# AkshayJha22/Cross-Sectional-Momentum-Strategy-Replication-Backtesting-Framework

Measured on AMD Instinct MI355X. Metric: asset-periods backtested/sec (1/2/4/8 GPU) + % HBM peak BW; decile match %, higher is better.
Workload: dtype f64

## Files before the change

cross-sectional-momentum-strategy-replication-backtesting-framework_amd/csrc/signal.hip:

```cpp
#include "csm_common.h"
#include "scan.h"
#include "shard.h"


#define PROBE_M 8
#define PROBE_DEN 8
__device__ __forceinline__ bool tail_probe(const double* __restrict__ P,
                                           const int64_t* __restrict__ month_start, int T_m,
                                           int64_t N, int64_t T_d) {
  static_assert(PROBE_M == 8, "the month spacing is a shift");
  const int lane = threadIdx.x & 63;
  const int64_t cs = N / 128;
  double x[PROBE_M][2];
  bool in[PROBE_M];
#pragma unroll
  for (int i = 0; i < PROBE_M; ++i) {
    const int m = (int)(((int64_t)(2 * i + 1) * T_m) >> 4);
    const int64_t d0 = month_start[m] < 0 ? 0 : month_start[m];
    const int64_t d1 = month_start[m + 1] < T_d ? month_start[m + 1] : T_d;
    in[i] = d1 > d0;
#pragma unroll
    for (int j = 0; j < 2; ++j)
      x[i][j] = in[i] ? P[(d1 - 1) * N + (2 * lane + j) * cs] : 0.0;
  }
  int gaps = 0, tot = 0;
#pragma unroll
  for (int i = 0; i < PROBE_M; ++i)
#pragma unroll
    for (int j = 0; j < 2; ++j) {
      gaps += __popcll(__ballot(in[i] && !(x[i][j] == x[i][j])));
      tot += in[i] ? 64 : 0;
    }
  return gaps * PROBE_DEN <= tot;
}

struct HaloArgs {
  int H, F, before, after;
  uint8_t* flags;
};
#define HALO_BATCH 8
template <int MAXD, int VEC, int NBUF, int BW, bool SH, bool BL, int JC = 0, bool HALO = false>
__global__ __launch_bounds__(64 * BW) void k_signal(
    const double* __restrict__ P, const int64_t* __restrict__ month_start, int T_m, int64_t N,
    int J, int skip, double* __restrict__ PMo, double* __restrict__ R, double* __restrict__ M,
    double* __restrict__ NR, const double* __restrict__ carry, const double* __restrict__ next_pm,
    double* __restrict__ carry_out, int64_t T_d, uint16_t* __restrict__ IDS, HaloArgs ha,
    int probe) {
  static_assert(!HALO || (SH && VEC == 2), "the halo prologue: shard passes, paired lanes");
  if (probe && tail_probe(P, month_start, T_m, N, T_d)) return;
  typedef typename RowT<VEC>::T VT;
  extern __shared__ __attribute__((aligned(16))) double ring_lds[];
  const int W = J + skip;
  const int tid = threadIdx.x;
  const int64_t a0 = ((int64_t)blockIdx.x * 64 * BW + tid) * VEC;
  const bool live = a0 < N;
  const int RS = 64 * VEC * BW;
  ScanLane sl[VEC];
  int* shc = reinterpret_cast<int*>(ring_lds + W * RS);
#pragma unroll
  for (int k = 0; k < VEC; ++k) {
    scan_init(sl[k], ring_lds + VEC * tid + k, RS, W, HALO ? nullptr : carry, N, a0 + k, live);
    if (SH) {
      shc[VEC * tid + k] = 0;
      shc[RS + VEC * tid + k] = -1;
      shc[2 * RS + VEC * tid + k] = -1;
    }
  }
  double npmh[VEC];
  if constexpr (HALO) {
    constexpr int HU = HALO_BATCH;
    const int64_t* ms = month_start;
    const int H = ha.H, F = ha.F, HF = H + F;
    const int64_t as = live ? a0 : 0;
    const int lane = tid & 63, wv = tid >> 6;
    const int64_t aw = a0 - 2 * lane;
    double* hpw = ring_lds + (size_t)W * RS + (size_t)(3 * RS) / 2;
    uint16_t* wl = reinterpret_cast<uint16_t*>(hpw + HU * RS) + wv * (HU * 128);
    int nh[VEC], fv[VEC], lv[VEC];
#pragma unroll
    for (int c = 0; c < VEC; ++c) { nh[c] = 0; fv[c] = -1; lv[c] = -1; npmh[c] = absent_val(); }
    for (int j0 = 0; j0 < HF; j0 += HU) {
      double2 xl[HU];
#pragma unroll
// ... 162 lines not shown
      }
    }
  };
  static_assert(NBUF == 2 || NBUF == 4, "two or four month buffers");
  VT A[MAXD], B[MAXD];
  if (NBUF == 2) {
    load_month(A, 0);
    for (int m = 0; m < T_m; m += 2) {
      load_month(B, m + 1);
      process(A, m);
      load_month(A, m + 2);
      if (m + 1 < T_m) process(B, m + 1);
    }
  } else {
    VT C[MAXD], D[MAXD];
    load_month(A, 0);
    load_month(B, 1);
    load_month(C, 2);
    for (int m = 0; m < T_m; m += 4) {
      load_month(D, m + 3);
      process(A, m);
      load_month(A, m + 4);
      if (m + 1 < T_m) process(B, m + 1);
      load_month(B, m + 5);
      if (m + 2 < T_m) process(C, m + 2);
      load_month(C, m + 6);
      if (m + 3 < T_m) process(D, m + 3);
    }
  }
  if (live) {
#pragma unroll
    for (int k = 0; k < VEC; ++k) {
      if constexpr (HALO) {
        if (sl[k].prev >= 0)
          NR[(int64_t)sl[k].prev * N + a0 + k] = pending_finish(npmh[k], sl[k].psff);
      } else {
        scan_finish(sl[k], ring_lds + VEC * tid + k, RS, W, N, a0 + k, NR, next_pm,
                    SH ? nullptr : carry_out);
      }
      if (SH) {
        const int* q = shc + VEC * tid + k;
        carry_out[a0 + k] = (double)q[0];
        carry_out[N + a0 + k] = (double)sl[k].prev;
        carry_out[2 * N + a0 + k] = sl[k].psff;
        carry_out[3 * N + a0 + k] = (double)q[RS];
        carry_out[4 * N + a0 + k] = (double)q[2 * RS];
      }
    }
  }
}

#define TAIL_U 8
#define TAIL_BACK 3

template <int MAXD, int BW, int JC>
__global__ __launch_bounds__(64 * BW) void k_signal_tail(
    const double* __restrict__ P, const int64_t* __restrict__ month_start, int T_m, int64_t N,
    int J, int skip, double* __restrict__ PMo, double* __restrict__ R, double* __restrict__ M,
    double* __restrict__ NR, const double* __restrict__ carry, const double* __restrict__ next_pm,
    double* __restrict__ carry_out, int64_t T_d, uint16_t* __restrict__ IDS,
    int probe) {
  if (probe && !tail_probe(P, month_start, T_m, N, T_d)) return;
  extern __shared__ __attribute__((aligned(16))) double ring_lds[];
  constexpr int U = TAIL_U, RS = 64 * BW, WA = 64;
  const int W = J + skip;
  const int tid = threadIdx.x, lane = tid & 63, wv = tid >> 6;
  const int64_t a0 = (int64_t)blockIdx.x * RS + tid;
  const bool live = a0 < N;
  const int64_t as = live ? a0 : 0;
  const int64_t aw = a0 - lane;
  const int64_t* ms = month_start;
  double* hp = ring_lds + (size_t)W * RS;
  double* hpw = hp + WA * wv;
  uint16_t* wl = reinterpret_cast<uint16_t*>(hp + U * RS) + wv * (2 * U * WA);
  uint16_t* wl2 = wl + U * WA;
  ScanLane sl;
  scan_init(sl, ring_lds + tid, RS, W, carry, N, a0, live);
  if (aw >= N) return;

  auto month_rows = [&](int m, int64_t& d0, int64_t& d1) {
    d0 = ms[m];
    d1 = ms[m + 1];
    d0 = d0 < 0 ? 0 : d0;
    d1 = d1 < T_d ? d1 : T_d;
  };
  auto load_last = [&](double (&xl)[U], int m0) {
#pragma unroll
    for (int u = 0; u < U; ++u) {
      xl[u] = absent_val();
      if (m0 + u < T_m) {
        int64_t d0, d1;
        month_rows(m0 + u, d0, d1);
        if (d1 > d0) xl[u] = P[(d1 - 1) * N + as];
      }
    }
  };
  auto fold = [&](double y, double& x, bool& got, bool& p) {
    if (!got && y == y) { x = y; got = true; }
    p |= !is_absent(y);
  };
  constexpr int K = MAXD - 1;
  struct Walk {
    int item, u, col;
    int64_t d0, d1;
    bool act;
  };
  auto issue = [&](auto& xs, Walk& w, const uint16_t* list, int it, int n, int m0) {
    constexpr int KK = sizeof(xs) / sizeof(double);
    w.act = it < n;
    w.item = w.act ? (int)list[it] : 0;
    w.u = w.item / WA;
    w.col = w.item % WA;
    month_rows(m0 + w.u, w.d0, w.d1);
    const int64_t a = aw + w.col;
#pragma unroll
    for (int k = 0; k < KK; ++k) {
      const int64_t d = w.d1 - 2 - k;
      xs[k] = (w.act && d >= w.d0) ? P[d * N + a] : absent_val();
    }
  };
  auto finish_back = [&](const double (&xs)[TAIL_BACK], const Walk& w, int& nb) {
    bool p = true, got = false;
    double x = 0.0;
#pragma unroll
    for (int k = 0; k < TAIL_BACK; ++k) fold(xs[k], x, got, p);
    const bool more = w.act && !got && w.d1 - 2 - TAIL_BACK >= w.d0;
    if (w.act && !more) hpw[w.u * RS + w.col] = got ? x : qnan();
    const uint64_t mk = __ballot(more);
    if (more) wl2[nb + lane_prefix(mk)] = (uint16_t)w.item;
    nb += __popcll(mk);
  };
  auto finish_month = [&](const double (&xs)[K], const Walk& w) {
    bool p = !is_absent(hpw[w.u * RS + w.col]), got = false;
    double x = 0.0;
#pragma unroll
    for (int k = 0; k < K; ++k) fold(xs[k], x, got, p);
    if (w.act) hpw[w.u * RS + w.col] = got ? x : (p ? qnan() : absent_val());
  };
  auto walk_months = [&](int i0, int n, int m0) {
    double XS[K], XT[K];
    Walk wb, wc;
    const bool two = i0 + 64 < n;
    issue(XS, wb, wl2, i0 + lane, n, m0);
    if (two) issue(XT, wc, wl2, i0 + 64 + lane, n, m0);
    finish_month(XS, wb);
    if (two) finish_month(XT, wc);
  };

  double xa[U], xb[U];
  load_last(xa, 0);
  for (int m0 = 0; m0 < T_m; m0 += U) {
    load_last(xb, m0 + U);
    int na = 0, nb = 0;
#pragma unroll
    for (int u = 0; u < U; ++u) {
      hp[u * RS + tid] = xa[u];
      bool in = false;
      if (m0 + u < T_m) {
        int64_t d0, d1;
        month_rows(m0 + u, d0, d1);
        in = d1 > d0;
      }
      const double x = xa[u];
      const bool need = live && in && !(x == x);
      const bool nb_ = need && is_absent(x), na_ = need && !nb_;
      const uint64_t mka = __ballot(na_), mkb = __ballot(nb_);
      const int item = u * WA + lane;
      if (na_) wl[na + lane_prefix(mka)] = (uint16_t)item;
      if (nb_) wl2[nb + lane_prefix(mkb)] = (uint16_t)item;
      na += __popcll(mka);
      nb += __popcll(mkb);
    }
    __builtin_amdgcn_wave_barrier();
    if (na + nb > 0) {
      double xs[TAIL_BACK];
      Walk wa;
      int db = nb < 128 ? nb : 128;
      issue(xs, wa, wl, lane, na, m0);
      walk_months(0, db, m0);
      finish_back(xs, wa, nb);
      for (int it0 = 64; it0 < na; it0 += 64) {
        issue(xs, wa, wl, it0 + lane, na, m0);
        finish_back(xs, wa, nb);
      }
      __builtin_amdgcn_wave_barrier();
      for (; db < nb; db += 128) walk_months(db, nb, m0);
    }
    __builtin_amdgcn_wave_barrier();
#pragma unroll 1
    for (int u = 0; u < U; ++u) {
      const int m = m0 + u;
      if (m >= T_m) break;
      if (!live) continue;
      const double pm = hp[u * RS + tid];
      if (PMo) PMo[(int64_t)m * N + a0] = pm;
      const double mom = scan_step<JC>(sl, pm, m, ring_lds + tid, RS, W, J, N, a0, R, M, NR);
      if (IDS) IDS[(int64_t)m * N + a0] = (uint16_t)csm_fid(mom);
    }
    __builtin_amdgcn_wave_barrier();
#pragma unroll
    for (int u = 0; u < U; ++u) xa[u] = xb[u];
  }
  if (live) scan_finish(sl, ring_lds + tid, RS, W, N, a0, NR, next_pm, carry_out);
}

static int g_tune_signal_vec = 2;
static int g_tune_signal_bwf = 0;
static int g_tune_signal_tail = 2;
static int g_tune_signal_j12 = 1;
#define SIGNAL_BWF_MIN_N (180 * 512)
static const TuneKnob g_knobs[] = {
    {"signal_vec", &g_tune_signal_vec, [](int v) { return v == 1 || v == 2; }},
    {"signal_bwf", &g_tune_signal_bwf, [](int v) { return v == 0 || v == 1 || v == 4; }},
    {"signal_j12", &g_tune_signal_j12, [](int v) { return v == 0 || v == 1; }},
    {"signal_tail", &g_tune_signal_tail, [](int v) { return v >= 0 && v <= 2; }},
};
int csm_tune_signal(const char* key, int value) { return tune_set(g_knobs, key, value); }

int signal_launch(csm_ctx* ctx, const char* who, const double* P, int64_t T_d, int64_t N,
                  const int64_t* month_start, int32_t T_m, int32_t max_month_days, int32_t J,
                  int32_t skip, double* PM, double* R, double* M, double* NR, const double* carry,
                  const double* next_pm, double* carry_out, bool sh, uint16_t* ids,
                  const HaloArgs* halo) {
  int r = prep(ctx);
  if (r) return r;
  if (sh && (!PM || !carry_out || T_m < 1))
    return set_err(ctx, CSM_E_INVAL, "%s: a shard pass needs PM and state, and at least one month",
                   who);
  if (!P || !month_start || !M || !NR || N <= 0 || T_d < 0 || T_m < 0 || J < 1 || skip < 0 ||
      J + skip > 256 || max_month_days < 1)
    return set_err(ctx, CSM_E_INVAL, "%s: bad arguments (N=%lld T_m=%d J=%d skip=%d)", who,
                   (long long)N, T_m, J, skip);
  if (max_month_days > 32)
    return set_err(ctx, CSM_E_INVAL, "%s: months longer than 32 days are not supported "
                   "(use csm_month_end + csm_momentum)", who);
  if (T_m == 0) return CSM_OK;
  if (T_d == 0)
    return set_err(ctx, CSM_E_INVAL, "%s: %d months and no day row", who, T_m);
  const int W = J + skip;
  const bool can2 = (N % 2 == 0) && aligned16(P) && (!PM || aligned16(PM)) && aligned16(M) &&
                    aligned16(NR) && (!R || aligned16(R));
  const int vec = (g_tune_signal_vec == 1 || !can2) ? 1 : 2;
  const size_t tlds = (size_t)(W + TAIL_U) * 128 * sizeof(double) + (size_t)2 * TAIL_U * 128 * sizeof(uint16_t);
  int tail = (!sh && !halo && can2 && tlds <= 160 * 1024) ? g_tune_signal_tail : 0;
  if (tail == 2 && N < (int64_t)SIGNAL_BWF_MIN_N) tail = 1;
  int probe_ = tail == 2;
  if (tail != 0) {
    const bool d23 = max_month_days <= 23, j12 = J == 12;
    const void* fn =
        d23 ? (j12 ? (const void*)k_signal_tail<23, 2, 12> : (const void*)k_signal_tail<23, 2, 0>)
            : (j12 ? (const void*)k_signal_tail<32, 2, 12> : (const void*)k_signal_tail<32, 2, 0>);
    if (tlds > 65536)
      HIP_CHECK(ctx, hipFuncSetAttribute(fn, hipFuncAttributeMaxDynamicSharedMemorySize, (int)tlds));
    const unsigned blocks = (unsigned)((N + 127) / 128);
    int T_m_ = T_m, J_ = J, skip_ = skip;
    int64_t N_ = N, T_d_ = T_d;
    void* args[] = {(void*)&P, (void*)&month_start, &T_m_, &N_, &J_, &skip_, (void*)&PM, (void*)&R,
                    (void*)&M, (void*)&NR, (void*)&carry, (void*)&next_pm, (void*)&carry_out, &T_d_,
                    (void*)&ids, &probe_};
    HIP_CHECK(ctx, hipLaunchKernel(fn, dim3(blocks), dim3(128), args, tlds, ctx->stream));
    LAUNCH_CHECK(ctx, who);
    if (tail == 1) return CSM_OK;
  }
  const bool fits4 = vec == 2 && max_month_days <= 23 && N * 8 * 32 < ((int64_t)1 << 31);
  const bool wide4 = fits4 && (g_tune_signal_bwf == 4 ||
                               (g_tune_signal_bwf == 0 && N >= (int64_t)SIGNAL_BWF_MIN_N));
  const int bw = wide4 ? 4 : 1;
  const size_t lds = (size_t)W * 64 * vec * bw * sizeof(double) +
                     (sh ? (size_t)3 * 64 * vec * bw * sizeof(int) : 0) +
                     (halo ? (size_t)HALO_BATCH * 64 * vec * bw * sizeof(double) +
                             (size_t)bw * HALO_BATCH * 128 * sizeof(uint16_t) : 0);
  const unsigned blocks = (unsigned)((N / vec + 64 * bw - 1) / (64 * bw));
  const void* fn = nullptr;
#define SIG1(V, SH_)                                                                            \
  (max_month_days <= 23 && V == 2 ? (const void*)k_signal<23, V, 4, 1, SH_, false>              \
   : max_month_days <= 24         ? (const void*)k_signal<24, V, 4, 1, SH_, false>              \
                                  : (const void*)k_signal<32, V, 4, 1, SH_, false>)
  const bool j12 = sh && J == 12 && g_tune_signal_j12;
  if (halo && !(sh && wide4))
    return set_err(ctx, CSM_E_INVAL, "%s: the fused halo prologue runs in the wide shard kernel "
                   "(even N >= %d, months of <= 23 days); use csm_shard_halo + "
                   "csm_signal_shard_halo", who, SIGNAL_BWF_MIN_N);
  if (halo)
    fn = j12 ? (const void*)k_signal<23, 2, 2, 4, true, true, 12, true>
             : (const void*)k_signal<23, 2, 2, 4, true, true, 0, true>;
  else if (wide4 && j12)
    fn = (const void*)k_signal<23, 2, 2, 4, true, true, 12>;
  else if (wide4)
    fn = sh ? (const void*)k_signal<23, 2, 2, 4, true, true> : (const void*)k_signal<23, 2, 2, 4, false, true>;
  else if (vec == 2)
    fn = sh ? SIG1(2, true) : SIG1(2, false);
  else
    fn = sh ? SIG1(1, true) : SIG1(1, false);
#undef SIG1
  if (lds > 65536)
    HIP_CHECK(ctx, hipFuncSetAttribute(fn, hipFuncAttributeMaxDynamicSharedMemorySize, (int)lds));
  {
    int T_m_ = T_m, J_ = J, skip_ = skip;
    int64_t N_ = N, T_d_ = T_d;
    HaloArgs ha = halo ? *halo : HaloArgs{0, 0, 0, 0, nullptr};
    void* args[] = {(void*)&P, (void*)&month_start, &T_m_, &N_, &J_, &skip_, (void*)&PM, (void*)&R,
                    (void*)&M, (void*)&NR, (void*)&carry, (void*)&next_pm, (void*)&carry_out, &T_d_,
                    (void*)&ids, (void*)&ha, &probe_};
    HIP_CHECK(ctx, hipLaunchKernel(fn, dim3(blocks), dim3(64 * bw), args, lds, ctx->stream));
  }
  LAUNCH_CHECK(ctx, who);
  return CSM_OK;
}

extern "C" {

int csm_signal(csm_ctx* ctx, const double* P, int64_t T_d, int64_t N, const int64_t* month_start,
               int32_t T_m, int32_t max_month_days, int32_t J, int32_t skip, double* PM, double* R,
// ... 65 lines not shown
```

cross-sectional-momentum-strategy-replication-backtesting-framework_amd/_lib.py:

```python
from __future__ import annotations

import ctypes
import os
from pathlib import Path

LIB_NAME = "libcsmom.so"
PKG_DIR = Path(__file__).resolve().parent
CSM_OK = 0
CSM_E_INVAL = -1
CSM_E_HIP = -2
CSM_E_RCCL = -3
CSM_E_TIMEOUT = -4
UNIQUE_ID_BYTES = 128
ABSENT_BITS = 0x7FF4000000000001

class CsmUnavailable(RuntimeError):
    """libcsmom.so is missing or failed to load (the engine has no CPU fallback)."""


class CsmError(RuntimeError):
    def __init__(self, status: int, msg: str):
        super().__init__(f"csmom status {status}: {msg}")
        self.status = status


def lib_path() -> Path:
    return Path(os.environ.get("CSMOM_LIB", PKG_DIR / LIB_NAME))


_LIB = None

_p = ctypes.c_void_p
_i32 = ctypes.c_int32
_i64 = ctypes.c_int64
_f64 = ctypes.c_double


SIGNATURES = {
    "csm_abi_version": (ctypes.c_int, []),
    "csm_tune": (ctypes.c_int, [ctypes.c_char_p, ctypes.c_int]),
    "csm_tune_ptr": (ctypes.c_int, [ctypes.c_char_p, _p]),
    "csm_create": (ctypes.c_int, [ctypes.c_int, ctypes.POINTER(ctypes.c_void_p)]),
    "csm_destroy": (ctypes.c_int, [_p]),
    "csm_last_error": (ctypes.c_char_p, [_p]),
    "csm_set_stream": (ctypes.c_int, [_p, _p]),
    "csm_sync": (ctypes.c_int, [_p]),
    "csm_month_end": (ctypes.c_int, [_p, _p, _p, _i64, _i64, _p, _i32, _p, _p]),
    "csm_momentum": (ctypes.c_int, [_p, _p, _i32, _i64, _i32, _i32, _p, _p, _p, _p, _p, _p]),
    "csm_momentum_multi": (ctypes.c_int, [_p, _p, _i32, _i64, _p, _i32, _i32, _p, _p]),
    "csm_momentum_multi_ids": (ctypes.c_int, [_p, _p, _i32, _i64, _p, _i32, _i32, _p, _p, _p]),
    "csm_signal": (ctypes.c_int, [_p, _p, _i64, _i64, _p, _i32, _i32, _i32, _i32, _p, _p, _p, _p,
                                  _p, _p, _p]),
    "csm_portfolio_workspace": (ctypes.c_int64, [_i32, _i32, _i64, _i32, _i32]),
    "csm_portfolio": (ctypes.c_int, [_p, _p, _p, _p, _i32, _i32, _i64, _i32, _i32, _f64, _f64,
                                     _f64, _p, _p, _p, _p, _p, _p, _p, _p]),
    "csm_cohort_sums": (ctypes.c_int, [_p, _p, _p, _p, _i32, _i32, _i64, _i32, _i32, _p]),
    "csm_portfolio_from_cohorts": (ctypes.c_int, [_p, _p, _p, _i32, _i32, _i64, _i32, _i32,
                                                  _i32, _f64, _f64, _f64, _p, _p, _p, _p,
                                                  _p, _p, _p, _p]),
    "csm_turnover_features": (ctypes.c_int, [_p, _p, _p, _p, _p, _i32, _i64, _i32, _p, _p, _p,
                                             _p]),
    "csm_double_sort_labels": (ctypes.c_int, [_p, _p, _p, _p, _p, _i32, _i64, _i32, _p, _p]),
    "csm_portfolio_from_cohorts_multi": (ctypes.c_int, [_p, _p, _p, _i32, _i32, _i64, _i32,
                                                        _i32, _i32, _p, _f64, _f64, _f64, _p,
                                                        _p, _p, _p, _p, _p, _p, _p]),
    "csm_cohort_sums_legs": (ctypes.c_int, [_p, _p, _p, _p, _i32, _i32, _i64, _i32, _i32, _p]),
    "csm_cohort_sums_js": (ctypes.c_int, [_p, _i32, _p, _p, _i32, _i32, _i64, _i32, _i32, _i32,
                                          _p]),
    "csm_portfolio_from_cohorts_legs": (ctypes.c_int, [_p, _p, _p, _i32, _i32, _i64, _i32,
                                                       _i32, _i32, _p, _f64, _f64, _f64, _p,
                                                       _p, _p, _p, _p, _p, _p, _p, _p]),
    "csm_cohort_sums_grouped": (ctypes.c_int, [_p, _i32, _p, _p, _p, _i32, _i32, _i64, _i32,
                                               _i32, _i32, _p]),
    "csm_cohort_sums_js_grouped": (ctypes.c_int, [_p, _i32, _p, _p, _i32, _i32, _i64, _i32,
                                                  _i32, _i32, _p]),
    "csm_portfolio_plan": (ctypes.c_int64, [_i32, _i32, _i64, _i32, _i32]),
    "csm_portfolio_from_cohorts_grouped": (ctypes.c_int, [_p, _i32, _p, _p, _i32, _i32, _i64,
                                                          _i32, _i32, _i32, _p, _f64, _f64, _f64,
                                                          _p, _p, _p, _p, _p, _p, _p, _p, _i32,
                                                          _p]),
    "csm_summary": (ctypes.c_int, [_p, _p, _p, _p, _p, _i32, _i32, _i32, _f64, _p]),
    "csm_daily_workspace": (ctypes.c_int64, [_i64, _i64, _i32, _i32, _i32]),
    "csm_daily_returns": (ctypes.c_int, [_p, _p, _i64, _i64, _p, _i32, _i32, _p, _p, _p, _i32,
                                         _i32, _p, _p, _p, _p]),
    "csm_series_stats": (ctypes.c_int, [_p, _p, _i32, _i32, _i64, _f64, _p]),
    "csm_month_stats": (ctypes.c_int, [_p, _p, _i64, _i64, _p, _i32, _i32, _p, _p, _p, _p, _p]),
    "csm_window_signals": (ctypes.c_int, [_p, _p, _p, _p, _p, _p, _p, _i32, _i64, _i32, _i32,
                                          _i32, _p, _p, _p, _p, _p, _p, _p]),
    "csm_market_factor": (ctypes.c_int, [_p, _p, _i32, _i64, _i32, _p, _p, _p]),
    "csm_market_model": (ctypes.c_int, [_p, _p, _p, _i32, _i64, _i32, _i32, _i32, _i32, _p, _p,
                                        _p, _p, _p]),
    "csm_next_ret": (ctypes.c_int, [_p, _p, _p, _i32, _i64, _p]),
    "csm_daily_market_workspace": (ctypes.c_int64, [_i64, _i64]),
    "csm_daily_market": (ctypes.c_int, [_p, _p, _i64, _i64, _i32, _i32, _p, _p, _p]),
# ... 119 lines not shown
```

cross-sectional-momentum-strategy-replication-backtesting-framework_amd/csrc/scan.h:

```cpp
#pragma once
#include "csm_common.h"

struct ScanLane {
  double pff;
  double psff;
  int head;
  int prev;
};

__device__ __forceinline__ void scan_init(ScanLane& s, double* ring, int RS, int W,
                                          const double* __restrict__ carry, int64_t N,
                                          int64_t a, bool live) {
  if (live && carry) {
    for (int k = 0; k < W; ++k) ring[k * RS] = carry[(int64_t)k * N + a];
    s.pff = carry[(int64_t)W * N + a];
    s.psff = carry[(int64_t)(W + 1) * N + a];
  } else {
    for (int k = 0; k < W; ++k) ring[k * RS] = qnan();
    s.pff = qnan();
    s.psff = qnan();
  }
  s.head = 0;
  s.prev = -1;
}
// ... 66 lines not shown
    return acc;
  }
  double acc = 1.0;
#pragma unroll
  for (int k = 0; k < RW; ++k) acc = (k >= lo && k < hi) ? acc * f[k] : acc;
  return acc;
}

__device__ __forceinline__ double subset_ret(double ps_new, double psff) {
  return ps_new / psff - 1.0;
}

template <class Settle>
__device__ __forceinline__ bool rank_step(double x, double mom, int m, double& psff, int& prev,
                                          Settle settle) {
  const bool ranked = !isnan_d(mom);
  const double ps_new = ffill(x, psff);
  if (prev >= 0) settle(prev, subset_ret(ps_new, psff));
  if (ranked) {
    psff = ps_new;
    prev = m;
    return false;
  }
  prev = -1;
  return true;
}

__device__ __forceinline__ double pending_finish(double x, double psff) {
  return is_absent(x) ? qnan() : subset_ret(ffill(x, psff), psff);
}

__device__ __forceinline__ void scan_finish(ScanLane& s, double* ring, int RS, int W, int64_t N,
                                            int64_t a, double* __restrict__ NR,
                                            const double* __restrict__ next_pm,
                                            double* __restrict__ carry_out) {
  if (s.prev >= 0)
    NR[(int64_t)s.prev * N + a] = next_pm ? pending_finish(next_pm[a], s.psff) : qnan();
  if (carry_out) {
    int idx = s.head;
    for (int k = 0; k < W; ++k) {
      carry_out[(int64_t)k * N + a] = ring[idx * RS];
      idx = (idx + 1 == W) ? 0 : idx + 1;
    }
    carry_out[(int64_t)W * N + a] = s.pff;
    carry_out[(int64_t)(W + 1) * N + a] = s.psff;
  }
}

template <int JC = 0>
__device__ __forceinline__ double lds_push_mom(ScanLane& s, double* ring, int RS, int W, int J,
                                               double fct) {
  lds_push(ring, RS, W, s.head, fct);
  return lds_prod<JC>(ring, RS, W, J, s.head) - 1.0;
}

template <class Ring>
__device__ __forceinline__ double scan_step_on(ScanLane& s, double x, int m, int64_t N, int64_t a,
                                               double* __restrict__ R, double* __restrict__ M,
                                               double* __restrict__ NR, Ring push_prod) {
  const double NaN = qnan();
  const int64_t o = (int64_t)m * N + a;
  if (is_absent(x)) {
    if (R) R[o] = NaN;
    M[o] = NaN;
    NR[o] = NaN;
    return NaN;
  }
  const double ret = price_step(x, s.pff);
  const double mom = push_prod(1.0 + ret);
  if (rank_step(x, mom, m, s.psff, s.prev,
                [&](int row, double nr) { NR[(int64_t)row * N + a] = nr; }))
    NR[o] = NaN;
  if (R) R[o] = ret;
  M[o] = mom;
  return mom;
}

__device__ __forceinline__ void store_pair(double* p, double v0, double v1) {
  *reinterpret_cast<double2*>(p) = make_double2(v0, v1);
}

__device__ __forceinline__ void store_next_ret_pair(double* __restrict__ NR, int64_t N,
                                                    int64_t a0, int64_t o, const int (&wp)[2],
                                                    const double (&vp)[2], const bool (&wc)[2]) {
  const double NaN = qnan();
  if (wp[0] >= 0 && wp[0] == wp[1]) {
    store_pair(NR + (int64_t)wp[0] * N + a0, vp[0], vp[1]);
  } else {
    if (wp[0] >= 0) NR[(int64_t)wp[0] * N + a0] = vp[0];
    if (wp[1] >= 0) NR[(int64_t)wp[1] * N + a0 + 1] = vp[1];
  }
  if (wc[0] && wc[1]) {
    store_pair(NR + o, NaN, NaN);
  } else {
    if (wc[0]) NR[o] = NaN;
    if (wc[1]) NR[o + 1] = NaN;
  }
}

__device__ __forceinline__ void chunk_range(int T_m, int G, int g, int& m0, int& m1) {
  const int base = T_m / G, rem = T_m % G;
  m0 = g * base + (g < rem ? g : rem);
  m1 = m0 + base + (g < rem ? 1 : 0);
}

template <int JC = 0>
// ... 18 lines not shown
  bool wc[2];
#pragma unroll
  for (int c = 0; c < 2; ++c) {
    wp[c] = -1;
    vp[c] = NaN;
    if (is_absent(x[c])) {
      ret[c] = NaN; mom[c] = NaN; wc[c] = true;
      continue;
    }
    ret[c] = price_step(x[c], s[c].pff);
    mom[c] = lds_push_mom<JC>(s[c], ring0 + c, RS, W, J, 1.0 + ret[c]);
    const bool ranked = !isnan_d(mom[c]);
    const double ps_new = ffill(x[c], s[c].psff);
    if (s[c].prev >= 0) { wp[c] = s[c].prev; vp[c] = subset_ret(ps_new, s[c].psff); }
    if (ranked) {
      s[c].psff = ps_new;
      s[c].prev = m;
      wc[c] = false;
    } else {
      s[c].prev = -1;
      wc[c] = true;
    }
  }
  const int64_t o = (int64_t)m * N + a0;
  if (R) store_pair(R + o, ret[0], ret[1]);
  store_pair(M + o, mom[0], mom[1]);
  store_next_ret_pair(NR, N, a0, o, wp, vp, wc);
}

__device__ __forceinline__ void scan_shadow(ScanLane& s, double x, int m, double* ring, int RS,
                                            int W, int J) {
  if (is_absent(x)) return;
  const double ret = price_step(x, s.pff);
  const double mom = lds_push_mom(s, ring, RS, W, J, 1.0 + ret);
  rank_step(x, mom, m, s.psff, s.prev, [](int, double) {});
}

template <int VEC> struct RowT;
template <> struct RowT<1> { typedef double T; };
template <> struct RowT<2> { typedef double2 T; };
__device__ __forceinline__ double comp(double v, int) { return v; }
__device__ __forceinline__ double comp(double2 v, int k) { return k == 0 ? v.x : v.y; }

template <int WR, int JC = 0>
__device__ __forceinline__ double scan_step_reg(ScanLane& s, double x, int m, double (&fr)[WR],
                                                int J, int64_t N, int64_t a,
                                                double* __restrict__ R, double* __restrict__ M,
                                                double* __restrict__ NR) {
  return scan_step_on(s, x, m, N, a, R, M, NR, [&](double fct) {
    reg_push(fr, fct);
    return reg_prod(fr, JC > 0 ? JC : J) - 1.0;
  });
}
```

include/csmom.h:

```cpp
#ifndef CSMOM_H
#define CSMOM_H

#include <stdint.h>

#ifdef __cplusplus
extern "C" {
#endif

#define CSM_ABI_VERSION 3
#define CSM_ABSENT_BITS 0x7FF4000000000001ULL

#define CSM_OK 0
#define CSM_E_INVAL (-1)
#define CSM_E_HIP (-2)
#define CSM_E_RCCL (-3)
#define CSM_E_TIMEOUT (-4)
#define CSM_UNIQUE_ID_BYTES 128

typedef struct csm_ctx csm_ctx;

int csm_abi_version(void);

int csm_tune(const char* key, int value);
int csm_tune_ptr(const char* key, void* p);

int csm_create(int device, csm_ctx** out);
int csm_destroy(csm_ctx* ctx);
const char* csm_last_error(const csm_ctx* ctx);
int csm_set_stream(csm_ctx* ctx, void* stream);
int csm_sync(csm_ctx* ctx);

int csm_month_end(csm_ctx* ctx, const double* P, const double* V, int64_t T_d, int64_t N,
                  const int64_t* month_start, int32_t T_m, double* PM, double* VOL);

int csm_momentum(csm_ctx* ctx, const double* PM, int32_t T_m, int64_t N, int32_t J,
                 int32_t skip, double* R, double* M, double* NR, const double* carry,
                 const double* next_pm, double* carry_out);

int csm_momentum_multi(csm_ctx* ctx, const double* PM, int32_t T_m, int64_t N,
                       const int32_t* Js, int32_t nJ, int32_t skip, double* const* M,
                       double* const* NR);
int csm_momentum_multi_ids(csm_ctx* ctx, const double* PM, int32_t T_m, int64_t N,
                           const int32_t* Js, int32_t nJ, int32_t skip, double* const* M,
                           double* const* NR, uint16_t* const* ids);

int64_t csm_momentum_chunked_workspace(int32_t T_m, int64_t N, int32_t J, int32_t skip,
                                       int32_t C);
int csm_momentum_chunked(csm_ctx* ctx, const double* PM, int32_t T_m, int64_t N, int32_t J,
                         int32_t skip, int32_t C, double* R, double* M, double* NR,
                         const double* next_pm, void* workspace);
int csm_momentum_chunked_ids(csm_ctx* ctx, const double* PM, int32_t T_m, int64_t N, int32_t J,
                             int32_t skip, int32_t C, double* R, double* M, double* NR,
                             const double* next_pm, uint16_t* ids, void* workspace);
int64_t csm_signal_chunked_workspace(int32_t T_m, int64_t N, int32_t J, int32_t skip, int32_t C);
int csm_signal_chunked(csm_ctx* ctx, const double* P, int64_t T_d, int64_t N,
                       const int64_t* month_start, int32_t T_m, int32_t max_month_days,
                       int32_t J, int32_t skip, int32_t C, double* R, double* M, double* NR,
                       uint16_t* ids, void* workspace);
int csm_signal_chunked_status(csm_ctx* ctx, void* workspace);
int64_t csm_momentum_multi_chunked_workspace(int32_t T_m, int64_t N, int32_t Jmax, int32_t skip,
                                             int32_t C);
int csm_momentum_multi_chunked(csm_ctx* ctx, const double* PM, int32_t T_m, int64_t N,
                               const int32_t* Js, int32_t nJ, int32_t skip, int32_t C,
                               double* const* M, double* const* NR, uint16_t* const* ids,
                               void* workspace);

int csm_signal(csm_ctx* ctx, const double* P, int64_t T_d, int64_t N, const int64_t* month_start,
               int32_t T_m, int32_t max_month_days, int32_t J, int32_t skip, double* PM,
               double* R, double* M, double* NR, const double* carry, const double* next_pm,
               double* carry_out);

int csm_signal_ids(csm_ctx* ctx, const double* P, int64_t T_d, int64_t N,
                   const int64_t* month_start, int32_t T_m, int32_t max_month_days,
                   int32_t min_month_days, int32_t J, int32_t skip, double* PM, double* R,
                   double* M, double* NR, uint16_t* ids);

// ... 243 lines not shown
```

Measured before the change: 796.9 billion.

## Prefetch tail month bounds and rows, make loads unconditional via spare-row redirection

Restructures the tail kernel's month loop so that the worklist for the next month group is built, and the bounds and last-row values two groups ahead are loaded, before the scan steps of the current group run. Loads overlap with scan work. Guarded loads are replaced by unconditional loads whose address falls back to a valid spare row, removing divergent branches around global reads. Month bounds are kept in a lane-distributed register and broadcast with shuffles instead of rereading month_start. The costs are higher register pressure from the extra prefetched arrays, and some redundant loads of the spare row.

Result: faster. 814.8 billion, median of 6 (+2.3%).

```diff
diff --git a/cross-sectional-momentum-strategy-replication-backtesting-framework_amd/csrc/signal.hip b/cross-sectional-momentum-strategy-replication-backtesting-framework_amd/csrc/signal.hip
--- a/cross-sectional-momentum-strategy-replication-backtesting-framework_amd/csrc/signal.hip
+++ b/cross-sectional-momentum-strategy-replication-backtesting-framework_amd/csrc/signal.hip
@@ -1,6 +1,7 @@
 #include "csm_common.h"
 #include "scan.h"
 #include "shard.h"
+#include "tailrows.h"
 
 
 #define PROBE_M 8
@@ -16,19 +17,17 @@
 #pragma unroll
   for (int i = 0; i < PROBE_M; ++i) {
     const int m = (int)(((int64_t)(2 * i + 1) * T_m) >> 4);
-    const int64_t d0 = month_start[m] < 0 ? 0 : month_start[m];
-    const int64_t d1 = month_start[m + 1] < T_d ? month_start[m + 1] : T_d;
+    const int64_t d0 = tail_bound(month_start[m], T_d), d1 = tail_bound(month_start[m + 1], T_d);
     in[i] = d1 > d0;
 #pragma unroll
-    for (int j = 0; j < 2; ++j)
-      x[i][j] = in[i] ? P[(d1 - 1) * N + (2 * lane + j) * cs] : 0.0;
+    for (int j = 0; j < 2; ++j) x[i][j] = P[tail_last_row(d1) * N + (2 * lane + j) * cs];
   }
   int gaps = 0, tot = 0;
 #pragma unroll
   for (int i = 0; i < PROBE_M; ++i)
 #pragma unroll
     for (int j = 0; j < 2; ++j) {
-      gaps += __popcll(__ballot(in[i] && !(x[i][j] == x[i][j])));
+      gaps += __popcll(__ballot(in[i] & !(x[i][j] == x[i][j])));
       tot += in[i] ? 64 : 0;
     }
   return gaps * PROBE_DEN <= tot;
@@ -323,90 +322,25 @@
   scan_init(sl, ring_lds + tid, RS, W, carry, N, a0, live);
   if (aw >= N) return;
 
-  auto month_rows = [&](int m, int64_t& d0, int64_t& d1) {
-    d0 = ms[m];
-    d1 = ms[m + 1];
-    d0 = d0 < 0 ? 0 : d0;
-    d1 = d1 < T_d ? d1 : T_d;
-  };
-  auto load_last = [&](double (&xl)[U], int m0) {
+  auto bounds = [&](int64_t (&c)[U + 1], int m0) {
+#pragma unroll
+    for (int u = 0; u <= U; ++u) c[u] = tail_bound(ms[m0 + u < T_m ? m0 + u : T_m], T_d);
+  };
+  auto load_last = [&](double (&xl)[U], const int64_t (&c)[U + 1]) {
+#pragma unroll
+    for (int u = 0; u < U; ++u) xl[u] = P[tail_last_row(c[u + 1]) * N + as];
+  };
+  int na = 0, nb = 0;
+  int64_t cv = 0;
+  int64_t spare = 0;
+  auto build = [&](const double (&xl)[U], const int64_t (&c)[U + 1]) {
+    na = nb = 0;
+    cv = c[U];
 #pragma unroll
     for (int u = 0; u < U; ++u) {
-      xl[u] = absent_val();
-      if (m0 + u < T_m) {
-        int64_t d0, d1;
-        month_rows(m0 + u, d0, d1);
-        if (d1 > d0) xl[u] = P[(d1 - 1) * N + as];
-      }
-    }
-  };
-  auto fold = [&](double y, double& x, bool& got, bool& p) {
-    if (!got && y == y) { x = y; got = true; }
-    p |= !is_absent(y);
-  };
-  constexpr int K = MAXD - 1;
-  struct Walk {
-    int item, u, col;
-    int64_t d0, d1;
-    bool act;
-  };
-  auto issue = [&](auto& xs, Walk& w, const uint16_t* list, int it, int n, int m0) {
-    constexpr int KK = sizeof(xs) / sizeof(double);
-    w.act = it < n;
-    w.item = w.act ? (int)list[it] : 0;
-    w.u = w.item / WA;
-    w.col = w.item % WA;
-    month_rows(m0 + w.u, w.d0, w.d1);
-    const int64_t a = aw + w.col;
-#pragma unroll
-    for (int k = 0; k < KK; ++k) {
-      const int64_t d = w.d1 - 2 - k;
-      xs[k] = (w.act && d >= w.d0) ? P[d * N + a] : absent_val();
-    }
-  };
-  auto finish_back = [&](const double (&xs)[TAIL_BACK], const Walk& w, int& nb) {
-    bool p = true, got = false;
-    double x = 0.0;
-#pragma unroll
-    for (int k = 0; k < TAIL_BACK; ++k) fold(xs[k], x, got, p);
-    const bool more = w.act && !got && w.d1 - 2 - TAIL_BACK >= w.d0;
-    if (w.act && !more) hpw[w.u * RS + w.col] = got ? x : qnan();
-    const uint64_t mk = __ballot(more);
-    if (more) wl2[nb + lane_prefix(mk)] = (uint16_t)w.item;
-    nb += __popcll(mk);
-  };
-  auto finish_month = [&](const double (&xs)[K], const Walk& w) {
-    bool p = !is_absent(hpw[w.u * RS + w.col]), got = false;
-    double x = 0.0;
-#pragma unroll
-    for (int k = 0; k < K; ++k) fold(xs[k], x, got, p);
-    if (w.act) hpw[w.u * RS + w.col] = got ? x : (p ? qnan() : absent_val());
-  };
-  auto walk_months = [&](int i0, int n, int m0) {
-    double XS[K], XT[K];
-    Walk wb, wc;
-    const bool two = i0 + 64 < n;
-    issue(XS, wb, wl2, i0 + lane, n, m0);
-    if (two) issue(XT, wc, wl2, i0 + 64 + lane, n, m0);
-    finish_month(XS, wb);
-    if (two) finish_month(XT, wc);
-  };
-
-  double xa[U], xb[U];
-  load_last(xa, 0);
-  for (int m0 = 0; m0 < T_m; m0 += U) {
-    load_last(xb, m0 + U);
-    int na = 0, nb = 0;
-#pragma unroll
-    for (int u = 0; u < U; ++u) {
-      hp[u * RS + tid] = xa[u];
-      bool in = false;
-      if (m0 + u < T_m) {
-        int64_t d0, d1;
-        month_rows(m0 + u, d0, d1);
-        in = d1 > d0;
-      }
-      const double x = xa[u];
+      const bool in = c[u + 1] > c[u];
+      const double x = in ? xl[u] : absent_val();
+      hp[u * RS + tid] = x;
       const bool need = live && in && !(x == x);
       const bool nb_ = need && is_absent(x), na_ = need && !nb_;
       const uint64_t mka = __ballot(na_), mkb = __ballot(nb_);
@@ -415,36 +349,104 @@
       if (nb_) wl2[nb + lane_prefix(mkb)] = (uint16_t)item;
       na += __popcll(mka);
       nb += __popcll(mkb);
-    }
+      cv = lane == u ? c[u] : cv;
+    }
+    spare = tail_last_row(c[1]);
     __builtin_amdgcn_wave_barrier();
+  };
+  auto fold = [&](double y, double& x, bool& got, bool& p) {
+    if (!got && y == y) { x = y; got = true; }
+    p |= !is_absent(y);
+  };
+  constexpr int K = MAXD - 1;
+  struct Walk {
+    int item, u, col, n;
+    int64_t d0, d1;
+    bool act;
+  };
+  auto issue = [&](auto& xs, Walk& w, const uint16_t* list, int it, int n) {
+    constexpr int KK = sizeof(xs) / sizeof(double);
+    w.act = it < n;
+    w.item = w.act ? (int)list[it] : 0;
+    w.u = w.item / WA;
+    w.col = w.item % WA;
+    w.d0 = __shfl(cv, w.u);
+    w.d1 = __shfl(cv, w.u + 1);
+    w.n = tail_walk_count(w.d0, w.d1, w.act, KK);
+    const int64_t a = aw + w.col;
+    const int64_t o1 = (w.d1 - 2) * N + a, os = spare * N + a;
+#pragma unroll
+    for (int k = 0; k < KK; ++k) xs[k] = P[tail_walk_off(o1, N, k, w.n, os)];
+  };
+  auto finish_back = [&](const double (&xs)[TAIL_BACK], const Walk& w, int& nb) {
+    bool p = true, got = false;
+    double x = 0.0;
+#pragma unroll
+    for (int k = 0; k < TAIL_BACK; ++k) fold(k < w.n ? xs[k] : absent_val(), x, got, p);
+    const bool more = w.act && !got && w.d1 - 2 - TAIL_BACK >= w.d0;
+    if (w.act && !more) hpw[w.u * RS + w.col] = got ? x : qnan();
+    const uint64_t mk = __ballot(more);
+    if (more) wl2[nb + lane_prefix(mk)] = (uint16_t)w.item;
+    nb += __popcll(mk);
+  };
+  auto finish_month = [&](const double (&xs)[K], const Walk& w) {
+    bool p = !is_absent(hpw[w.u * RS + w.col]), got = false;
+    double x = 0.0;
+#pragma unroll
+    for (int k = 0; k < K; ++k) fold(k < w.n ? xs[k] : absent_val(), x, got, p);
+    if (w.act) hpw[w.u * RS + w.col] = got ? x : (p ? qnan() : absent_val());
+  };
+  auto walk_months = [&](int i0, int n) {
+    double XS[K], XT[K];
+    Walk wb, wc;
+    issue(XS, wb, wl2, i0 + lane, n);
+    if (i0 + 64 < n) {
+      issue(XT, wc, wl2, i0 + 64 + lane, n);
+      finish_month(XT, wc);
+    }
+    finish_month(XS, wb);
+  };
+
+  int64_t c[U + 1];
+  double x[U], pmr[U];
+  bounds(c, 0);
+  load_last(x, c);
+  build(x, c);
+  bounds(c, U);
+  load_last(x, c);
+  for (int m0 = 0; m0 < T_m; m0 += U) {
     if (na + nb > 0) {
       double xs[TAIL_BACK];
       Walk wa;
       int db = nb < 128 ? nb : 128;
-      issue(xs, wa, wl, lane, na, m0);
-      walk_months(0, db, m0);
+      issue(xs, wa, wl, lane, na);
+      walk_months(0, db);
       finish_back(xs, wa, nb);
       for (int it0 = 64; it0 < na; it0 += 64) {
-        issue(xs, wa, wl, it0 + lane, na, m0);
+        issue(xs, wa, wl, it0 + lane, na);
         finish_back(xs, wa, nb);
       }
       __builtin_amdgcn_wave_barrier();
-      for (; db < nb; db += 128) walk_months(db, nb, m0);
+      for (; db < nb; db += 128) walk_months(db, nb);
     }
     __builtin_amdgcn_wave_barrier();
+#pragma unroll
+    for (int u = 0; u < U; ++u) pmr[u] = hp[u * RS + tid];
+    build(x, c);
+    bounds(c, m0 + 2 * U);
+    load_last(x, c);
 #pragma unroll 1
     for (int u = 0; u < U; ++u) {
       const int m = m0 + u;
       if (m >= T_m) break;
       if (!live) continue;
-      const double pm = hp[u * RS + tid];
+      double pm = pmr[0];
+#pragma unroll
+      for (int k = 1; k < U; ++k) pm = u == k ? pmr[k] : pm;
       if (PMo) PMo[(int64_t)m * N + a0] = pm;
       const double mom = scan_step<JC>(sl, pm, m, ring_lds + tid, RS, W, J, N, a0, R, M, NR);
       if (IDS) IDS[(int64_t)m * N + a0] = (uint16_t)csm_fid(mom);
     }
-    __builtin_amdgcn_wave_barrier();
-#pragma unroll
-    for (int u = 0; u < U; ++u) xa[u] = xb[u];
   }
   if (live) scan_finish(sl, ring_lds + tid, RS, W, N, a0, NR, next_pm, carry_out);
 }
diff --git a/cross-sectional-momentum-strategy-replication-backtesting-framework_amd/csrc/tailrows.h b/cross-sectional-momentum-strategy-replication-backtesting-framework_amd/csrc/tailrows.h
--- /dev/null
+++ b/cross-sectional-momentum-strategy-replication-backtesting-framework_amd/csrc/tailrows.h
@@ -0,0 +1,21 @@
+#pragma once
+#include <cstdint>
+
+#if defined(__HIPCC__) || defined(__CUDACC__)
+#define TR_HD __host__ __device__ __forceinline__
+#else
+#define TR_HD inline
+#endif
+
+TR_HD int64_t tail_bound(int64_t ms, int64_t T_d) { return ms < 0 ? 0 : (ms < T_d ? ms : T_d); }
+
+TR_HD int64_t tail_last_row(int64_t d1) { return d1 > 0 ? d1 - 1 : 0; }
+
+TR_HD int tail_walk_count(int64_t d0, int64_t d1, bool active, int cap) {
+  const int64_t n = d1 - 1 - d0;
+  return (!active || n <= 0) ? 0 : (n < (int64_t)cap ? (int)n : cap);
+}
+
+TR_HD int64_t tail_walk_off(int64_t o1, int64_t stride, int k, int n, int64_t spare) {
+  return k < n ? o1 - (int64_t)k * stride : spare;
+}
```

## Restructure signal tail kernel to single-wave blocks with adaptive lanes and register ring

Applied to the files above, without the earlier changes.

The tail signal kernel now launches one-wave blocks whose number of active lanes per block is chosen from occupancy queries, so small-N cross sections spread over more CUs. For J=12, skip=1 the momentum ring lives in registers instead of LDS, and the LDS ring uses an offset-based push. Month bounds are staged in LDS and the back-walk loads are made branchless. The cost is partially idle lanes per wave, a cached occupancy query on the host, and more register pressure in the register-ring variant.

Measured after the change: 831.4 billion before, 884.8 billion after, median of 6. 1.06x the previous value.

```diff
diff --git a/cross-sectional-momentum-strategy-replication-backtesting-framework_amd/_lib.py b/cross-sectional-momentum-strategy-replication-backtesting-framework_amd/_lib.py
--- a/cross-sectional-momentum-strategy-replication-backtesting-framework_amd/_lib.py
+++ b/cross-sectional-momentum-strategy-replication-backtesting-framework_amd/_lib.py
@@ -40,6 +40,7 @@
     "csm_abi_version": (ctypes.c_int, []),
     "csm_tune": (ctypes.c_int, [ctypes.c_char_p, ctypes.c_int]),
     "csm_tune_ptr": (ctypes.c_int, [ctypes.c_char_p, _p]),
+    "csm_signal_tail_lanes": (ctypes.c_int, [_i64, ctypes.c_int]),
     "csm_create": (ctypes.c_int, [ctypes.c_int, ctypes.POINTER(ctypes.c_void_p)]),
     "csm_destroy": (ctypes.c_int, [_p]),
     "csm_last_error": (ctypes.c_char_p, [_p]),
diff --git a/cross-sectional-momentum-strategy-replication-backtesting-framework_amd/csrc/scan.h b/cross-sectional-momentum-strategy-replication-backtesting-framework_amd/csrc/scan.h
--- a/cross-sectional-momentum-strategy-replication-backtesting-framework_amd/csrc/scan.h
+++ b/cross-sectional-momentum-strategy-replication-backtesting-framework_amd/csrc/scan.h
@@ -142,6 +142,28 @@
                                                double fct) {
   lds_push(ring, RS, W, s.head, fct);
   return lds_prod<JC>(ring, RS, W, J, s.head) - 1.0;
+}
+
+template <int JC = 0>
+__device__ __forceinline__ double lds_off_push_mom(double* ring, int RS, int WRS, int J, int& off,
+                                                   double fct) {
+  ring[off] = fct;
+  off = (off + RS == WRS) ? 0 : off + RS;
+  auto slot = [&](int k) {
+    const unsigned t = (unsigned)(off + k * RS);
+    return ring[min(t, t - (unsigned)WRS)];
+  };
+  double acc = slot(0);
+  if constexpr (JC > 0) {
+    double f[JC];
+#pragma unroll
+    for (int k = 1; k < JC; ++k) f[k] = slot(k);
+#pragma unroll
+    for (int k = 1; k < JC; ++k) acc = acc * f[k];
+  } else {
+    for (int k = 1; k < J; ++k) acc = acc * slot(k);
+  }
+  return acc - 1.0;
 }
 
 template <class Ring>
@@ -266,3 +288,30 @@
     return reg_prod(fr, JC > 0 ? JC : J) - 1.0;
   });
 }
+
+template <int WR>
+__device__ __forceinline__ void scan_init_reg(ScanLane& s, double (&fr)[WR],
+                                              const double* __restrict__ carry, int64_t N,
+                                              int64_t a, bool live) {
+  const bool in = live && carry;
+#pragma unroll
+  for (int k = 0; k < WR; ++k) fr[k] = in ? carry[(int64_t)k * N + a] : qnan();
+  s.pff = in ? carry[(int64_t)WR * N + a] : qnan();
+  s.psff = in ? carry[(int64_t)(WR + 1) * N + a] : qnan();
+  s.head = 0;
+  s.prev = -1;
+}
+template <int WR>
+__device__ __forceinline__ void scan_finish_reg(const ScanLane& s, const double (&fr)[WR],
+                                                int64_t N, int64_t a, double* __restrict__ NR,
+                                                const double* __restrict__ next_pm,
+                                                double* __restrict__ carry_out) {
+  if (s.prev >= 0)
+    NR[(int64_t)s.prev * N + a] = next_pm ? pending_finish(next_pm[a], s.psff) : qnan();
+  if (carry_out) {
+#pragma unroll
+    for (int k = 0; k < WR; ++k) carry_out[(int64_t)k * N + a] = fr[k];
+    carry_out[(int64_t)WR * N + a] = s.pff;
+    carry_out[(int64_t)(WR + 1) * N + a] = s.psff;
+  }
+}
diff --git a/cross-sectional-momentum-strategy-replication-backtesting-framework_amd/csrc/signal.hip b/cross-sectional-momentum-strategy-replication-backtesting-framework_amd/csrc/signal.hip
--- a/cross-sectional-momentum-strategy-replication-backtesting-framework_amd/csrc/signal.hip
+++ b/cross-sectional-momentum-strategy-replication-backtesting-framework_amd/csrc/signal.hip
@@ -297,116 +297,123 @@
 
 #define TAIL_U 8
 #define TAIL_BACK 3
-
-template <int MAXD, int BW, int JC>
-__global__ __launch_bounds__(64 * BW) void k_signal_tail(
+#define TAIL_MAX_W 148
+
+static size_t tail_lds_bytes(int ring_rows, int la) {
+  return (size_t)(ring_rows + TAIL_U) * la * sizeof(double) + (TAIL_U + 1) * sizeof(int64_t) +
+         (size_t)2 * TAIL_U * la * sizeof(uint16_t);
+}
+
+template <int MAXD, int WR, int JC>
+__global__ __launch_bounds__(64) void k_signal_tail(
     const double* __restrict__ P, const int64_t* __restrict__ month_start, int T_m, int64_t N,
     int J, int skip, double* __restrict__ PMo, double* __restrict__ R, double* __restrict__ M,
     double* __restrict__ NR, const double* __restrict__ carry, const double* __restrict__ next_pm,
     double* __restrict__ carry_out, int64_t T_d, uint16_t* __restrict__ IDS,
-    int probe) {
+    int probe, int LA) {
   if (probe && !tail_probe(P, month_start, T_m, N, T_d)) return;
   extern __shared__ __attribute__((aligned(16))) double ring_lds[];
-  constexpr int U = TAIL_U, RS = 64 * BW, WA = 64;
-  const int W = J + skip;
-  const int tid = threadIdx.x, lane = tid & 63, wv = tid >> 6;
-  const int64_t a0 = (int64_t)blockIdx.x * RS + tid;
-  const bool live = a0 < N;
-  const int64_t as = live ? a0 : 0;
-  const int64_t aw = a0 - lane;
+  constexpr int U = TAIL_U, WA = 64;
+  const int W = J + skip, RS = LA, WRS = W * RS;
+  const int lane = threadIdx.x;
+  const int64_t aw = (int64_t)blockIdx.x * LA;
+  const int64_t a0 = aw + lane;
+  const bool own = lane < LA;
+  const bool live = own && a0 < N;
+  const int64_t as = live ? a0 : aw;
   const int64_t* ms = month_start;
-  double* hp = ring_lds + (size_t)W * RS;
-  double* hpw = hp + WA * wv;
-  uint16_t* wl = reinterpret_cast<uint16_t*>(hp + U * RS) + wv * (2 * U * WA);
-  uint16_t* wl2 = wl + U * WA;
+  double* hp = ring_lds + (WR > 0 ? 0 : WRS);
+  int64_t* mb = reinterpret_cast<int64_t*>(hp + U * RS);
+  uint16_t* wl = reinterpret_cast<uint16_t*>(mb + U + 1);
+  uint16_t* wl2 = wl + U * RS;
   ScanLane sl;
-  scan_init(sl, ring_lds + tid, RS, W, carry, N, a0, live);
-  if (aw >= N) return;
-
-  auto month_rows = [&](int m, int64_t& d0, int64_t& d1) {
-    d0 = ms[m];
-    d1 = ms[m + 1];
-    d0 = d0 < 0 ? 0 : d0;
-    d1 = d1 < T_d ? d1 : T_d;
-  };
-  auto load_last = [&](double (&xl)[U], int m0) {
-#pragma unroll
-    for (int u = 0; u < U; ++u) {
-      xl[u] = absent_val();
-      if (m0 + u < T_m) {
-        int64_t d0, d1;
-        month_rows(m0 + u, d0, d1);
-        if (d1 > d0) xl[u] = P[(d1 - 1) * N + as];
-      }
-    }
-  };
-  auto fold = [&](double y, double& x, bool& got, bool& p) {
-    if (!got && y == y) { x = y; got = true; }
-    p |= !is_absent(y);
+  double fr[WR > 0 ? WR : 1];
+  int ho = 0;
+  if constexpr (WR > 0) {
+    scan_init_reg(sl, fr, carry, N, a0, live);
+  } else {
+    sl.pff = sl.psff = qnan();
+    sl.head = 0;
+    sl.prev = -1;
+    if (own) scan_init(sl, ring_lds + lane, RS, W, carry, N, a0, live);
+  }
+
+  auto bound = [&](int i) {
+    const int64_t d = ms[i < T_m ? i : T_m];
+    return d < 0 ? 0 : (d < T_d ? d : T_d);
+  };
+  auto load_last = [&](double (&xl)[U], int64_t (&c)[U + 1], int m0) {
+#pragma unroll
+    for (int u = 0; u <= U; ++u) c[u] = bound(m0 + u);
+#pragma unroll
+    for (int u = 0; u < U; ++u) xl[u] = P[(c[u + 1] > 0 ? c[u + 1] - 1 : 0) * N + as];
+#pragma unroll
+    for (int u = 0; u < U; ++u) xl[u] = c[u + 1] > c[u] ? xl[u] : absent_val();
   };
   constexpr int K = MAXD - 1;
   struct Walk {
-    int item, u, col;
-    int64_t d0, d1;
+    int item, cell, rows;
     bool act;
   };
-  auto issue = [&](auto& xs, Walk& w, const uint16_t* list, int it, int n, int m0) {
+  auto issue = [&](auto& xs, Walk& w, const uint16_t* list, int it, int n) {
     constexpr int KK = sizeof(xs) / sizeof(double);
     w.act = it < n;
     w.item = w.act ? (int)list[it] : 0;
-    w.u = w.item / WA;
-    w.col = w.item % WA;
-    month_rows(m0 + w.u, w.d0, w.d1);
-    const int64_t a = aw + w.col;
+    const int u = w.item / WA, col = w.item % WA;
+    w.cell = __mul24(u, RS) + col;
+    const int64_t d0 = w.act ? mb[u] : 0, d1 = w.act ? mb[u + 1] : 1;
+    w.rows = (int)(d1 - 1 - d0);
+    int64_t i = (d1 - 1) * N + aw + col;
 #pragma unroll
     for (int k = 0; k < KK; ++k) {
-      const int64_t d = w.d1 - 2 - k;
-      xs[k] = (w.act && d >= w.d0) ? P[d * N + a] : absent_val();
-    }
+      i -= k < w.rows ? N : 0;
+      xs[k] = P[i];
+    }
+  };
+  auto fold = [&](double y, bool in, double& x, bool& got, bool& p) {
+    if (in && !got && y == y) { x = y; got = true; }
+    p |= in && !is_absent(y);
   };
   auto finish_back = [&](const double (&xs)[TAIL_BACK], const Walk& w, int& nb) {
     bool p = true, got = false;
     double x = 0.0;
 #pragma unroll
-    for (int k = 0; k < TAIL_BACK; ++k) fold(xs[k], x, got, p);
-    const bool more = w.act && !got && w.d1 - 2 - TAIL_BACK >= w.d0;
-    if (w.act && !more) hpw[w.u * RS + w.col] = got ? x : qnan();
+    for (int k = 0; k < TAIL_BACK; ++k) fold(xs[k], k < w.rows, x, got, p);
+    const bool more = w.act && !got && w.rows > TAIL_BACK;
+    if (w.act && !more) hp[w.cell] = got ? x : qnan();
     const uint64_t mk = __ballot(more);
     if (more) wl2[nb + lane_prefix(mk)] = (uint16_t)w.item;
     nb += __popcll(mk);
   };
   auto finish_month = [&](const double (&xs)[K], const Walk& w) {
-    bool p = !is_absent(hpw[w.u * RS + w.col]), got = false;
+    bool p = w.act && !is_absent(hp[w.act ? w.cell : 0]), got = false;
     double x = 0.0;
 #pragma unroll
-    for (int k = 0; k < K; ++k) fold(xs[k], x, got, p);
-    if (w.act) hpw[w.u * RS + w.col] = got ? x : (p ? qnan() : absent_val());
-  };
-  auto walk_months = [&](int i0, int n, int m0) {
-    double XS[K], XT[K];
-    Walk wb, wc;
-    const bool two = i0 + 64 < n;
-    issue(XS, wb, wl2, i0 + lane, n, m0);
-    if (two) issue(XT, wc, wl2, i0 + 64 + lane, n, m0);
+    for (int k = 0; k < K; ++k) fold(xs[k], k < w.rows, x, got, p);
+    if (w.act) hp[w.cell] = got ? x : (p ? qnan() : absent_val());
+  };
+  auto walk_months = [&](int i0, int n) {
+    double XS[K];
+    Walk wb;
+    issue(XS, wb, wl2, i0 + lane, n);
     finish_month(XS, wb);
-    if (two) finish_month(XT, wc);
   };
 
   double xa[U], xb[U];
-  load_last(xa, 0);
+  int64_t ca[U + 1], cb[U + 1];
+  load_last(xa, ca, 0);
   for (int m0 = 0; m0 < T_m; m0 += U) {
-    load_last(xb, m0 + U);
+    load_last(xb, cb, m0 + U);
+    if (lane == 0) {
+#pragma unroll
+      for (int u = 0; u <= U; ++u) mb[u] = ca[u];
+    }
     int na = 0, nb = 0;
 #pragma unroll
     for (int u = 0; u < U; ++u) {
-      hp[u * RS + tid] = xa[u];
-      bool in = false;
-      if (m0 + u < T_m) {
-        int64_t d0, d1;
-        month_rows(m0 + u, d0, d1);
-        in = d1 > d0;
-      }
       const double x = xa[u];
+      if (own) hp[u * RS + lane] = x;
+      const bool in = ca[u + 1] > ca[u];
       const bool need = live && in && !(x == x);
       const bool nb_ = need && is_absent(x), na_ = need && !nb_;
       const uint64_t mka = __ballot(na_), mkb = __ballot(nb_);
@@ -420,38 +427,62 @@
     if (na + nb > 0) {
       double xs[TAIL_BACK];
       Walk wa;
-      int db = nb < 128 ? nb : 128;
-      issue(xs, wa, wl, lane, na, m0);
-      walk_months(0, db, m0);
+      int db = nb < 64 ? nb : 64;
+      issue(xs, wa, wl, lane, na);
+      walk_months(0, db);
       finish_back(xs, wa, nb);
       for (int it0 = 64; it0 < na; it0 += 64) {
-        issue(xs, wa, wl, it0 + lane, na, m0);
+        issue(xs, wa, wl, it0 + lane, na);
         finish_back(xs, wa, nb);
       }
       __builtin_amdgcn_wave_barrier();
-      for (; db < nb; db += 128) walk_months(db, nb, m0);
+      for (; db < nb; db += 64) walk_months(db, nb);
     }
     __builtin_amdgcn_wave_barrier();
+    const int nu = live ? (T_m - m0 < U ? T_m - m0 : U) : 0;
 #pragma unroll 1
-    for (int u = 0; u < U; ++u) {
+    for (int u = 0; u < nu; ++u) {
       const int m = m0 + u;
-      if (m >= T_m) break;
-      if (!live) continue;
-      const double pm = hp[u * RS + tid];
+      const double pm = hp[u * RS + lane];
       if (PMo) PMo[(int64_t)m * N + a0] = pm;
-      const double mom = scan_step<JC>(sl, pm, m, ring_lds + tid, RS, W, J, N, a0, R, M, NR);
+      double mom;
+      if constexpr (WR > 0) {
+        double fnew = 0.0;
+        mom = scan_step_on(sl, pm, m, N, a0, R, M, NR, [&](double fct) {
+          double g[WR];
+#pragma unroll
+          for (int k = 0; k + 1 < WR; ++k) g[k] = fr[k + 1];
+          g[WR - 1] = fnew = fct;
+          return reg_prod(g, JC > 0 ? JC : J) - 1.0;
+        });
+        reg_push(fr, fnew, !is_absent(pm));
+      } else
+        mom = scan_step_on(sl, pm, m, N, a0, R, M, NR, [&](double fct) {
+          return lds_off_push_mom<JC>(ring_lds + lane, RS, WRS, J, ho, fct);
+        });
       if (IDS) IDS[(int64_t)m * N + a0] = (uint16_t)csm_fid(mom);
     }
     __builtin_amdgcn_wave_barrier();
 #pragma unroll
     for (int u = 0; u < U; ++u) xa[u] = xb[u];
-  }
-  if (live) scan_finish(sl, ring_lds + tid, RS, W, N, a0, NR, next_pm, carry_out);
+#pragma unroll
+    for (int u = 0; u <= U; ++u) ca[u] = cb[u];
+  }
+  if (live) {
+    if constexpr (WR > 0) {
+      scan_finish_reg(sl, fr, N, a0, NR, next_pm, carry_out);
+    } else {
+      sl.head = ho / RS;
+      scan_finish(sl, ring_lds + lane, RS, W, N, a0, NR, next_pm, carry_out);
+    }
+  }
 }
 
 static int g_tune_signal_vec = 2;
 static int g_tune_signal_bwf = 0;
 static int g_tune_signal_tail = 2;
+static int g_tune_signal_tail_lanes = 0;
+static int g_tune_signal_tail_reg = 1;
 static int g_tune_signal_j12 = 1;
 #define SIGNAL_BWF_MIN_N (180 * 512)
 static const TuneKnob g_knobs[] = {
@@ -459,8 +490,40 @@
     {"signal_bwf", &g_tune_signal_bwf, [](int v) { return v == 0 || v == 1 || v == 4; }},
     {"signal_j12", &g_tune_signal_j12, [](int v) { return v == 0 || v == 1; }},
     {"signal_tail", &g_tune_signal_tail, [](int v) { return v >= 0 && v <= 2; }},
+    {"signal_tail_lanes", &g_tune_signal_tail_lanes, [](int v) { return v >= 0 && v <= 64 && v % 8 == 0; }},
+    {"signal_tail_reg", &g_tune_signal_tail_reg, [](int v) { return v == 0 || v == 1; }},
 };
 int csm_tune_signal(const char* key, int value) { return tune_set(g_knobs, key, value); }
+
+extern "C" int csm_signal_tail_lanes(int64_t N, int capacity) {
+  const int64_t room = (int64_t)capacity - capacity / 32;
+  for (int la = 8; la < 64; la += 8)
+    if ((N + la - 1) / la <= room) return la;
+  return 64;
+}
+
+#define TAIL_SIMDS_PER_CU 4
+static int tail_lanes_auto(csm_ctx* ctx, const void* fn, int ring_rows, int64_t N, int* la_out) {
+  static struct { const void* fn; int ring_rows, device, la; int64_t N; } memo = {nullptr, 0, 0, 0, 0};
+  if (memo.fn == fn && memo.ring_rows == ring_rows && memo.device == ctx->device && memo.N == N) {
+    *la_out = memo.la;
+    return CSM_OK;
+  }
+  const int n_cu = ctx->n_cu > 0 ? ctx->n_cu : 256;
+  int la = 8;
+  for (;;) {
+    int per_cu = 0;
+    HIP_CHECK(ctx, hipOccupancyMaxActiveBlocksPerMultiprocessor(&per_cu, fn, 64,
+                                                                tail_lds_bytes(ring_rows, la)));
+    const int need = csm_signal_tail_lanes(N, per_cu * n_cu);
+    if (need <= la || la == 64) break;
+    la = need;
+  }
+  while (la < 64 && (N + la - 1) / la > (int64_t)TAIL_SIMDS_PER_CU * n_cu) la += 8;
+  memo = {fn, ring_rows, ctx->device, la, N};
+  *la_out = la;
+  return CSM_OK;
+}
 
 int signal_launch(csm_ctx* ctx, const char* who, const double* P, int64_t T_d, int64_t N,
                   const int64_t* month_start, int32_t T_m, int32_t max_month_days, int32_t J,
@@ -486,24 +549,33 @@
   const bool can2 = (N % 2 == 0) && aligned16(P) && (!PM || aligned16(PM)) && aligned16(M) &&
                     aligned16(NR) && (!R || aligned16(R));
   const int vec = (g_tune_signal_vec == 1 || !can2) ? 1 : 2;
-  const size_t tlds = (size_t)(W + TAIL_U) * 128 * sizeof(double) + (size_t)2 * TAIL_U * 128 * sizeof(uint16_t);
-  int tail = (!sh && !halo && can2 && tlds <= 160 * 1024) ? g_tune_signal_tail : 0;
+  int tail = (!sh && !halo && can2 && W <= TAIL_MAX_W) ? g_tune_signal_tail : 0;
   if (tail == 2 && N < (int64_t)SIGNAL_BWF_MIN_N) tail = 1;
   int probe_ = tail == 2;
   if (tail != 0) {
-    const bool d23 = max_month_days <= 23, j12 = J == 12;
+    const bool d23 = max_month_days <= 23, j12 = J == 12, reg = j12 && skip == 1 && g_tune_signal_tail_reg;
     const void* fn =
-        d23 ? (j12 ? (const void*)k_signal_tail<23, 2, 12> : (const void*)k_signal_tail<23, 2, 0>)
-            : (j12 ? (const void*)k_signal_tail<32, 2, 12> : (const void*)k_signal_tail<32, 2, 0>);
-    if (tlds > 65536)
-      HIP_CHECK(ctx, hipFuncSetAttribute(fn, hipFuncAttributeMaxDynamicSharedMemorySize, (int)tlds));
-    const unsigned blocks = (unsigned)((N + 127) / 128);
+        d23 ? (reg   ? (const void*)k_signal_tail<23, 13, 12>
+               : j12 ? (const void*)k_signal_tail<23, 0, 12> : (const void*)k_signal_tail<23, 0, 0>)
+            : (reg   ? (const void*)k_signal_tail<32, 13, 12>
+               : j12 ? (const void*)k_signal_tail<32, 0, 12> : (const void*)k_signal_tail<32, 0, 0>);
+    const int ring_rows = reg ? 0 : W;
+    if (tail_lds_bytes(ring_rows, 64) > 65536)
+      HIP_CHECK(ctx, hipFuncSetAttribute(fn, hipFuncAttributeMaxDynamicSharedMemorySize,
+                                         (int)tail_lds_bytes(ring_rows, 64)));
+    int LA_ = g_tune_signal_tail_lanes;
+    if (LA_ == 0) {
+      r = tail_lanes_auto(ctx, fn, ring_rows, N, &LA_);
+      if (r) return r;
+    }
+    const size_t tlds = tail_lds_bytes(ring_rows, LA_);
+    const unsigned blocks = (unsigned)((N + LA_ - 1) / LA_);
     int T_m_ = T_m, J_ = J, skip_ = skip;
     int64_t N_ = N, T_d_ = T_d;
     void* args[] = {(void*)&P, (void*)&month_start, &T_m_, &N_, &J_, &skip_, (void*)&PM, (void*)&R,
                     (void*)&M, (void*)&NR, (void*)&carry, (void*)&next_pm, (void*)&carry_out, &T_d_,
-                    (void*)&ids, &probe_};
-    HIP_CHECK(ctx, hipLaunchKernel(fn, dim3(blocks), dim3(128), args, tlds, ctx->stream));
+                    (void*)&ids, &probe_, &LA_};
+    HIP_CHECK(ctx, hipLaunchKernel(fn, dim3(blocks), dim3(64), args, tlds, ctx->stream));
     LAUNCH_CHECK(ctx, who);
     if (tail == 1) return CSM_OK;
   }
diff --git a/include/csmom.h b/include/csmom.h
--- a/include/csmom.h
+++ b/include/csmom.h
@@ -22,6 +22,7 @@
 int csm_abi_version(void);
 
 int csm_tune(const char* key, int value);
+int csm_signal_tail_lanes(int64_t N, int capacity);
 int csm_tune_ptr(const char* key, void* p);
 
 int csm_create(int device, csm_ctx** out);
```
